# maxwerhahn/Multi-pass-GAN

Measured on AMD Instinct MI355X. Metric: volumes/sec (4x two-pass generator inference, 64^3->256^3 density-only), higher is better.
Workload: dtype f16+2xbf6->f32

## Files before the change

### multi-pass-gan_amd/csrc/mpgan_conv.h

```cpp
#pragma once
#include "mpgan_internal.h"
#include "mpgan_mfma_dev.h"

namespace mpg::conv {

using namespace mpg::dev;

constexpr int TW = 32;
constexpr int TAPOFF_BYTES = 1024;
constexpr int epi_rowf(int nt) { return nt * 32 + 4; }

struct SegArgs {
    const char* x;
    const char* w;
    int cg_seg;
    int cg_total, g_off;
    int kh, kw, up;
    int cgc, nchunks, sc;
    int ih, iw;
    int pt, pl;
    int hs, ws;
    int np;
    int ni_img;
    int direct;
    int tp;
    int pref;
};

struct ConvArgs {
    int n, h, w, cout, nseg;
    SegArgs seg[MPG_MAX_SEG];
    const float* bias;
    int act;
    float leak;
    int pn;
    float pn_eps;
    const float* post_add;
    int pa_stride, pa_coff;
    float* y;
    char* y_g8;
    const float* in_amax;
    const char* zeros;
    int img_bytes;
    int tap_bytes;
    int tiles_x, tiles_y;
    int dbg;
};

typedef const __attribute__((address_space(4))) ConvArgs* KArgs;

struct ConvArgsD2S {
    ConvArgs a;
    int cs;
    int coff;
    int cg;
};
typedef const __attribute__((address_space(4))) ConvArgsD2S* KArgsD2S;

template <bool D2S>
struct KernelArgs { typedef ConvArgs type; };
template <>
struct KernelArgs<true> { typedef ConvArgsD2S type; };

struct D2SPos {
    int cc;
    size_t pix;
};
__device__ __forceinline__ D2SPos d2s_pos(const KArgsD2S dp, int py, int px, int c) {
    const int gc = dp->coff + c;
    const int k = gc / dp->cs;
    D2SPos p;
    p.cc = gc - k * dp->cs;
    p.pix = (size_t)(2 * py + (k >> 1)) * (2 * dp->a.w) + 2 * px + (k & 1);
    return p;
}

template <int NT, int PREC>
struct Pipe {
    static constexpr int WAVES = 4;
    static constexpr int NPL = (PREC == 3) ? 2 : 1;
    static constexpr int PT = (NT >= 3) ? 2 : 4;
    static constexpr int TH = 4 * PT;
    static constexpr int KS = (PREC == 3) ? ((NT == 4 || NT == 2) ? 1 : 2) : ((NT == 4 || NT == 2) ? 2 : 4);
    static constexpr int R = (NT == 3) ? 3 : 4;
    static constexpr int D = R - 1;
    static constexpr int WPLANE = KS * NT * 1024;
    static constexpr int WSTAGE = WPLANE * NPL;
    static constexpr int NI = WSTAGE / 4096;
    static constexpr int ROWF = epi_rowf(NT);
    static_assert(WSTAGE % 4096 == 0, "stage must be a whole number of 256 x 16-byte pieces");
};

template <int NT>
struct Pipe6 {
    static constexpr int WAVES = (NT == 1) ? 4 : 8;
    static constexpr int PT = 16 / WAVES;
    static constexpr int TH = 16;
    static constexpr int KS = 4;
    static constexpr int WF16 = KS * NT * 1024;
    static constexpr int WF6 = NT * 2048;
    static constexpr int WSTAGE = WF16 + 2 * WF6;
    static constexpr int R = 3;
    static constexpr int D = R - 1;
    static constexpr int NI = WSTAGE / (WAVES * 1024);
    static constexpr int ROWF = epi_rowf(NT);
    static_assert(WSTAGE % (WAVES * 1024) == 0, "stage must be a whole number of per-wave pieces");
};

struct EpiPre {
    float bias;
    float amax;
};
__device__ __forceinline__ EpiPre epilogue_prefetch(const KArgs ap, int tid) {
    const auto& a = *ap;
    EpiPre pre;
    pre.bias = (a.bias != nullptr && tid < a.cout) ? a.bias[tid] : 0.f;
    pre.amax = a.in_amax != nullptr ? *a.in_amax : 0.f;
    return pre;
}

template <int ACT, int NT>
__device__ __forceinline__ void epilogue_bias_act(f32x16 (&acc)[NT], const float* bl, float* stg_lane, float unscale, float leak, int cout,
                                                  int hh) {
    if constexpr (ACT == MPG_ACT_TANH) {
#pragma unroll
        for (int nt = 0; nt < NT; ++nt)
#pragma unroll
            for (int q4 = 0; q4 < 4; ++q4) {
                const int co0 = nt * 32 + 8 * q4 + 4 * hh;
                const float4 bq = *reinterpret_cast<const float4*>(bl + co0);
                *reinterpret_cast<float4*>(stg_lane + co0) =
                    make_float4(acc[nt][4 * q4] * unscale + bq.x, acc[nt][4 * q4 + 1] * unscale + bq.y,
                                acc[nt][4 * q4 + 2] * unscale + bq.z, acc[nt][4 * q4 + 3] * unscale + bq.w);
            }
#pragma nounroll
        for (int k = 0; k < NT * 16; ++k) {
            const int c = (k >> 2) * 8 + 4 * hh + (k & 3);
            stg_lane[c] = c < cout ? tanhf(stg_lane[c]) : 0.f;
        }
#pragma unroll
        for (int nt = 0; nt < NT; ++nt)
#pragma unroll
            for (int q4 = 0; q4 < 4; ++q4) {
                const float4 v = *reinterpret_cast<const float4*>(stg_lane + nt * 32 + 8 * q4 + 4 * hh);
                acc[nt][4 * q4] = v.x;
                acc[nt][4 * q4 + 1] = v.y;
                acc[nt][4 * q4 + 2] = v.z;
                acc[nt][4 * q4 + 3] = v.w;
            }
        return;
    }
    float4 bq[2][4];
#pragma unroll
    for (int q4 = 0; q4 < 4; ++q4) bq[0][q4] = *reinterpret_cast<const float4*>(bl + 8 * q4 + 4 * hh);
#pragma unroll
    for (int nt = 0; nt < NT; ++nt) {
        if (nt + 1 < NT) {
#pragma unroll
            for (int q4 = 0; q4 < 4; ++q4) bq[(nt + 1) & 1][q4] = *reinterpret_cast<const float4*>(bl + (nt + 1) * 32 + 8 * q4 + 4 * hh);
        }
        __builtin_amdgcn_sched_barrier(0);
#pragma unroll
        for (int q4 = 0; q4 < 4; ++q4) {
            const int co0 = nt * 32 + 8 * q4 + 4 * hh;
            const float b4[4] = {bq[nt & 1][q4].x, bq[nt & 1][q4].y, bq[nt & 1][q4].z, bq[nt & 1][q4].w};
#pragma unroll
            for (int i = 0; i < 4; ++i) {
                float v = mpg::apply_act(acc[nt][4 * q4 + i] * unscale + b4[i], ACT, leak);
                if (co0 + i >= cout) v = 0.f;
                acc[nt][4 * q4 + i] = v;
            }
        }
        __builtin_amdgcn_sched_barrier(0);
    }
}

template <int NT>
__device__ __forceinline__ void epilogue_row_values(f32x16 (&acc)[NT], const KArgs ap, const float* bl, float* stg_lane, float unscale,
                                                    int hh) {
    const auto& a = *ap;
    switch (a.act) {
        case MPG_ACT_RELU: epilogue_bias_act<MPG_ACT_RELU>(acc, bl, stg_lane, unscale, a.leak, a.cout, hh); break;
        case MPG_ACT_LRELU: epilogue_bias_act<MPG_ACT_LRELU>(acc, bl, stg_lane, unscale, a.leak, a.cout, hh); break;
        case MPG_ACT_TANH: epilogue_bias_act<MPG_ACT_TANH>(acc, bl, stg_lane, unscale, a.leak, a.cout, hh); break;
        default: epilogue_bias_act<MPG_ACT_NONE>(acc, bl, stg_lane, unscale, a.leak, a.cout, hh); break;
    }
    if (a.pn) {
        float ss = 0.f;
#pragma unroll
        for (int nt = 0; nt < NT; ++nt)
#pragma unroll
            for (int i = 0; i < 16; ++i) ss += acc[nt][i] * acc[nt][i];
        ss += __shfl_xor(ss, 32);
        const float sc = rsqrtf(ss / (float)a.cout + a.pn_eps);
#pragma unroll
        for (int nt = 0; nt < NT; ++nt)
#pragma unroll
            for (int i = 0; i < 16; ++i) acc[nt][i] *= sc;
    }
}

template <int NT, int PT, bool D2S = false>
__device__ __forceinline__ void conv_epilogue(f32x16 (&acc)[PT][NT], const KArgs ap, char* smem, int n, int y0, int x0,
                                              int wave, int lane, const EpiPre pre) {
    const auto& a = *ap;
    const KArgsD2S dp = reinterpret_cast<KArgsD2S>(ap);
    const int r = lane & 31;
    const int hh = lane >> 5;
    constexpr int ROWF = epi_rowf(NT);
    static_assert(128 * sizeof(float) <= TAPOFF_BYTES, "the staged bias must fit in front of the staging rows");
    float* bl = reinterpret_cast<float*>(smem);
    float* stg = reinterpret_cast<float*>(smem + TAPOFF_BYTES) + wave * (32 * ROWF);
    const int cg_out = (a.cout + 7) >> 3;
    const float unscale = 1.f / mpg::pow2_scale(pre.amax);
    {
        float bv = pre.bias;
        asm volatile("" : "+v"(bv));
        if (wave < 2) bl[wave * 64 + lane] = bv;
    }
    __syncthreads();
    const int npx = min(32, a.w - x0);
    const size_t plane_px = (size_t)a.h * a.w;
    if (a.y == nullptr && a.post_add == nullptr) {
#pragma unroll
        for (int pt = 0; pt < PT; ++pt) {
            const int py = y0 + PT * wave + pt;
            epilogue_row_values<NT>(acc[pt], ap, bl, stg + r * ROWF, unscale, hh);
            if (py < a.h && r < npx && !(a.dbg & 2)) {
#pragma unroll
                for (int nt = 0; nt < NT; ++nt)
#pragma unroll
                    for (int qp = 0; qp < 2; ++qp) {
                        float v[8];
#pragma unroll
                        for (int i = 0; i < 4; ++i) {
                            typedef unsigned v2u_t __attribute__((ext_vector_type(2)));
                            const v2u_t sw = __builtin_amdgcn_permlane32_swap(__float_as_uint(acc[pt][nt][8 * qp + i]),
                                                                              __float_as_uint(acc[pt][nt][8 * qp + 4 + i]), false, false);
                            v[i] = __uint_as_float(sw[0]);
                            v[4 + i] = __uint_as_float(sw[1]);
                        }
                        const int cg = nt * 4 + 2 * qp + hh;
                        if (cg < cg_out) {
                            char* dst;
                            size_t plane_out = plane_px;
                            if constexpr (D2S) {
                                const D2SPos q = d2s_pos(dp, py, x0 + r, 8 * cg);
                                plane_out = 4 * plane_px;
                                dst = a.y_g8 + ((((size_t)n * dp->cg + (q.cc >> 3)) * 2) * plane_out + q.pix) * 16;
                            } else {
                                dst = a.y_g8 + ((((size_t)n * cg_out + cg) * 2) * plane_px + (size_t)py * a.w + x0 + r) * 16;
                            }
                            half8 hi, lo;
#pragma unroll
                            for (int j = 0; j < 8; ++j) {
                                hi[j] = (_Float16)v[j];
                                lo[j] = (_Float16)(v[j] - (float)hi[j]);
                            }
                            __builtin_nontemporal_store(hi, reinterpret_cast<half8*>(dst));
                            __builtin_nontemporal_store(lo, reinterpret_cast<half8*>(dst + plane_out * 16));
                        }
                    }
            }
        }
        return;
    }
#pragma unroll
    for (int pt = 0; pt < PT; ++pt) {
        const int py = y0 + PT * wave + pt;
        epilogue_row_values<NT>(acc[pt], ap, bl, stg + r * ROWF, unscale, hh);
#pragma unroll
        for (int nt = 0; nt < NT; ++nt)
#pragma unroll
            for (int q4 = 0; q4 < 4; ++q4) {
                const int co0 = nt * 32 + 8 * q4 + 4 * hh;
                *reinterpret_cast<float4*>(stg + r * ROWF + co0) =
                    make_float4(acc[pt][nt][4 * q4], acc[pt][nt][4 * q4 + 1], acc[pt][nt][4 * q4 + 2], acc[pt][nt][4 * q4 + 3]);
            }
        if (py < a.h && !(a.dbg & 2)) {
            const size_t pix0 = ((size_t)n * a.h + py) * a.w + x0;
            if (a.post_add != nullptr) {
                const float* pa = a.post_add + pix0 * a.pa_stride + a.pa_coff;
                const int total = npx * a.cout;
                for (int f0 = lane; f0 < total; f0 += 256) {
                    float pv[4];
                    int so[4];
#pragma unroll
                    for (int j = 0; j < 4; ++j) {
                        const int f = min(f0 + 64 * j, total - 1);
                        const int p = f / a.cout;
                        const int c = f - p * a.cout;
                        so[j] = p * ROWF + c;
                        pv[j] = pa[(size_t)p * a.pa_stride + c];
                    }
#pragma unroll
                    for (int j = 0; j < 4; ++j) {
                        asm volatile("" : "+v"(pv[j]));
                        if (f0 + 64 * j < total) stg[so[j]] += pv[j];
                    }
                }
            }
            if (D2S && a.y != nullptr) {
                float* img = a.y + (size_t)n * 4 * a.h * a.w * dp->cs;
                const int total = npx * a.cout;
                if (((dp->cs | dp->coff | a.cout) & 3) == 0) {
                    for (int f = lane * 4; f < total; f += 256) {
                        const int p = f / a.cout;
                        const int c = f - p * a.cout;
                        const D2SPos q = d2s_pos(dp, py, x0 + p, c);
                        *reinterpret_cast<float4*>(img + q.pix * dp->cs + q.cc) = *reinterpret_cast<const float4*>(stg + p * ROWF + c);
                    }
                } else {
                    for (int f = lane; f < total; f += 64) {
                        const int p = f / a.cout;
                        const int c = f - p * a.cout;
                        const D2SPos q = d2s_pos(dp, py, x0 + p, c);
                        img[q.pix * dp->cs + q.cc] = stg[p * ROWF + c];
                    }
                }
            } else if (a.y != nullptr) {
                float* dst = a.y + pix0 * a.cout;
                const int total = npx * a.cout;
                if ((a.cout & 3) == 0) {
                    for (int f = lane * 4; f < total; f += 256) {
                        const int p = f / a.cout;
                        const int c = f - p * a.cout;
                        *reinterpret_cast<float4*>(dst + f) = *reinterpret_cast<const float4*>(stg + p * ROWF + c);
                    }
                } else {
                    for (int f = lane; f < total; f += 64) {
                        const int p = f / a.cout;
                        dst[f] = stg[p * ROWF + (f - p * a.cout)];
                    }
                }
            }
            if (a.y_g8 != nullptr) {
                if (r < npx) {
                    for (int cg = hh; cg < cg_out; cg += 2) {
                        const float4 v0 = *reinterpret_cast<const float4*>(stg + r * ROWF + cg * 8);
                        const float4 v1 = *reinterpret_cast<const float4*>(stg + r * ROWF + cg * 8 + 4);
                        const float v[8] = {v0.x, v0.y, v0.z, v0.w, v1.x, v1.y, v1.z, v1.w};
                        char* dst;
                        size_t plane_out = plane_px;
                        if constexpr (D2S) {
                            const D2SPos q = d2s_pos(dp, py, x0 + r, 8 * cg);
                            plane_out = 4 * plane_px;
                            dst = a.y_g8 + ((((size_t)n * dp->cg + (q.cc >> 3)) * 2) * plane_out + q.pix) * 16;
                        } else {
                            dst = a.y_g8 + ((((size_t)n * cg_out + cg) * 2) * plane_px + (size_t)py * a.w + x0 + r) * 16;
                        }
                        half8 hi, lo;
#pragma unroll
                        for (int j = 0; j < 8; ++j) {
                            hi[j] = (_Float16)v[j];
                            lo[j] = (_Float16)(v[j] - (float)hi[j]);
                        }
                        __builtin_nontemporal_store(hi, reinterpret_cast<half8*>(dst));
                        __builtin_nontemporal_store(lo, reinterpret_cast<half8*>(dst + plane_out * 16));
                    }
                }
            }
        }
    }
}

struct Shape {
    int th;
    int ks;
    int waves;
    int wstage;
    int ring;
    int rowf;
};
const Shape& pipe_shape(int nt, int prec);

struct SegShape {
    int cgc, nchunks, sc, np, ni_img, img_bytes, direct, tp, pref;
    int slots;
    int stages;
};
SegShape seg_shape(int kh, int kw, int cin, int nt, int prec);

constexpr size_t LDS_MAX = 160 * 1024;

size_t pack_base_bytes(int kh, int kw, int cin, int cout, int prec);
inline bool small_layer(int cin, int cout) { return cin <= 8 && cout <= 8; }
inline int pad_before(int k, int pad_hi) { return pad_hi ? k / 2 : (k - 1) / 2; }
int check_segment(const mpg_conv_desc* d, int s);

hipError_t launch_conv_f16(int prec, int nt, dim3 grid, size_t lds, hipStream_t st, const ConvArgs& a);
hipError_t launch_conv_f16(int prec, int nt, dim3 grid, size_t lds, hipStream_t st, const ConvArgsD2S& a);
hipError_t launch_conv_f6(int nt, dim3 grid, size_t lds, hipStream_t st, const ConvArgs& a);
int launch_small(hipStream_t stream, const mpg_conv_desc* d);

}
```

### multi-pass-gan_amd/csrc/mpgan_conv_f6.hip

```cpp
#include "mpgan_conv.h"

using namespace mpg::conv;

namespace {

#ifndef MPG_AH
#define MPG_AH 2
#endif
#ifndef MPG_WD
#define MPG_WD 1
#endif
#ifndef MPG_DIAG6
#define MPG_DIAG6 0
#endif
#ifndef MPG_W0
#define MPG_W0 1
#endif
#ifndef MPG_IMG_LATE
#define MPG_IMG_LATE 0
#endif
#ifndef MPG_PIECES_AFTER
#define MPG_PIECES_AFTER 1
#endif
#ifndef MPG_ALT
#define MPG_ALT 0
#endif
#ifndef MPG_STAMPS
#define MPG_STAMPS 0
#endif
#if MPG_STAMPS
#define MPG_STAMP(v) asm volatile("s_memtime %0" : "=s"(v))
#else
#define MPG_STAMP(v)
#endif
constexpr int lo_step(int pt, int nt, int ptn) {
    const int s = nt - ptn + pt - 1;
    return s < 0 ? 0 : (s > nt - 1 ? nt - 1 : s);
}

typedef int v16i __attribute__((ext_vector_type(16)));
typedef int v8i __attribute__((ext_vector_type(8)));
typedef int v6i __attribute__((ext_vector_type(6)));
typedef _Float16 half32 __attribute__((ext_vector_type(32)));
typedef _Float16 half16 __attribute__((ext_vector_type(16)));

__device__ __forceinline__ v8i lds_read32(const char* p) {
    const v4i lo = *reinterpret_cast<const v4i*>(p);
    const v4i hi = *reinterpret_cast<const v4i*>(p + 1024);
    return __builtin_shufflevector(lo, hi, 0, 1, 2, 3, 4, 5, 6, 7);
}

template <int OFF, class T>
__device__ __forceinline__ void ds_read16(T& dst, unsigned addr) {
    static_assert(sizeof(T) == 16 && OFF >= 0 && OFF < 65536, "one ds_read_b128");
    asm volatile("ds_read_b128 %0, %1 offset:%2" : "=v"(dst) : "v"(addr), "n"(OFF));
}

constexpr int kx_cum(int h, int NT, int PT) { return h + PT * ((h + NT - 1) / NT); }
constexpr int kx_allowed(int g, int NT, int PT, int AH) {
    const int G16 = 4 * NT;
    const int hi = g + AH + 1 < G16 ? g + AH + 1 : G16;
    return kx_cum(hi, NT, PT) - kx_cum(g + 1, NT, PT);
}

__device__ __forceinline__ half32 cat32(const half8& a, const half8& b, const half8& c, const half8& d) {
    const half16 lo = __builtin_shufflevector(a, b, 0, 1, 2, 3, 4, 5, 6, 7, 8, 9, 10, 11, 12, 13, 14, 15);
    const half16 hi = __builtin_shufflevector(c, d, 0, 1, 2, 3, 4, 5, 6, 7, 8, 9, 10, 11, 12, 13, 14, 15);
    return __builtin_shufflevector(lo, hi, 0, 1, 2, 3, 4, 5, 6, 7, 8, 9, 10, 11, 12, 13, 14, 15, 16, 17, 18, 19, 20, 21, 22, 23,
                                   24, 25, 26, 27, 28, 29, 30, 31);
}

__device__ __forceinline__ int block_exp16(const half32& v) {
    const v16i r = __builtin_bit_cast(v16i, v);
    int a0, a1, a2, a3, a4, a5, a6, a7, b0, b1, b2, b3, b4, b5, b6, b7, m2, m1;
#define MPG_MAX3(d, x, y, z) asm("v_pk_maximum3_f16 %0, %1, %2, %3" : "=v"(d) : "v"(x), "v"(y), "v"(z))
#define MPG_MIN3(d, x, y, z) asm("v_pk_minimum3_f16 %0, %1, %2, %3" : "=v"(d) : "v"(x), "v"(y), "v"(z))
    MPG_MAX3(a0, r[0], r[1], r[2]); MPG_MAX3(a1, r[3], r[4], r[5]); MPG_MAX3(a2, r[6], r[7], r[8]); MPG_MAX3(a3, r[9], r[10], r[11]);
    MPG_MAX3(a4, r[12], r[13], r[14]); MPG_MAX3(a5, a0, a1, r[15]); MPG_MAX3(a6, a2, a3, a4); MPG_MAX3(a7, a5, a6, a6);
    MPG_MIN3(b0, r[0], r[1], r[2]); MPG_MIN3(b1, r[3], r[4], r[5]); MPG_MIN3(b2, r[6], r[7], r[8]); MPG_MIN3(b3, r[9], r[10], r[11]);
    MPG_MIN3(b4, r[12], r[13], r[14]); MPG_MIN3(b5, b0, b1, r[15]); MPG_MIN3(b6, b2, b3, b4); MPG_MIN3(b7, b5, b6, b6);
#undef MPG_MAX3
#undef MPG_MIN3
    asm("v_pk_max_f16 %0, %1, %2 neg_lo:[0,1] neg_hi:[0,1]" : "=v"(m2) : "v"(a7), "v"(b7));
    asm("v_pk_max_f16 %0, %1, %1 op_sel:[0,1] op_sel_hi:[1,0]" : "=v"(m1) : "v"(m2));
    return (m1 >> 10) & 31;
}

#ifndef MPG_CVT_DIVIDES
#define MPG_CVT_DIVIDES 1
#endif
__device__ __forceinline__ float pow2_from_byte(int e8m0) {
#if MPG_CVT_DIVIDES
    return __builtin_bit_cast(float, e8m0 << 23);
#else
    return __builtin_bit_cast(float, (254 - e8m0) << 23);
#endif
}
__device__ __forceinline__ v8i widen6(const v6i& v) {
    return __builtin_shufflevector(v, v, 0, 1, 2, 3, 4, 5, -1, -1);
}
__device__ __forceinline__ v8i bf6_of(const half32& v, int e8m0) {
    return widen6(__builtin_amdgcn_cvt_scalef32_pk32_bf6_f16(v, pow2_from_byte(e8m0)));
}
constexpr int BF6 = 3;

template <int NT>
__global__ __launch_bounds__(Pipe6<NT>::WAVES * 64, 2) void conv_mfma_f6_kernel(const ConvArgs a_unused) {
    extern __shared__ __attribute__((aligned(16))) char smem[];
    const KArgs ap = (KArgs)__builtin_amdgcn_kernarg_segment_ptr();
    const auto& a = *ap;
    using P = Pipe6<NT>;
    constexpr int WAVES = P::WAVES, PT = P::PT, TH = P::TH, WF16 = P::WF16, WF6 = P::WF6, WSTAGE = P::WSTAGE;
    constexpr int NI = P::NI, R = P::R, D = P::D, THREADS = WAVES * 64;

    int* tap16 = reinterpret_cast<int*>(smem);
    char* img_lds = smem + a.tap_bytes;
    char* w_lds = img_lds + 2 * a.img_bytes;

    const int tid = threadIdx.x;
    const int lane = tid & 63;
    const int wave = tid >> 6;
    const int wave_u = __builtin_amdgcn_readfirstlane(wave);
    const int r = lane & 31;
    const int hh = lane >> 5;

    int bid = blockIdx.x;
    const int nblk = gridDim.x;
    if ((nblk & 7) == 0) bid = (bid & 7) * (nblk >> 3) + (bid >> 3);
    const int tx = bid % a.tiles_x;
    const int t2 = bid / a.tiles_x;
    const int ty = t2 % a.tiles_y;
    const int n = t2 / a.tiles_y;
    const int y0 = ty * TH, x0 = tx * TW;

    f32x16 acc[PT][NT];
#pragma unroll
    for (int pt = 0; pt < PT; ++pt)
#pragma unroll
        for (int nt = 0; nt < NT; ++nt)
#pragma unroll
            for (int i = 0; i < 16; ++i) acc[pt][nt][i] = 0.f;

    const EpiPre pre = epilogue_prefetch(ap, tid);
    const int seg_flip = (NT == 1 && a.nseg > 1) ? ((int)(blockIdx.x >> 8) & 1) : 0;
    for (int s0 = 0; s0 < ((a.dbg & 1) ? 0 : a.nseg); ++s0) {
        const int s = seg_flip ? a.nseg - 1 - s0 : s0;
        const auto& sg = ap->seg[s];
        if (NT <= 2 && sg.direct) {
            const unsigned plane_bytes = (unsigned)(sg.hs * sg.ws) * 16u;
            const unsigned gstride = 2u * plane_bytes;
            const char* xb = sg.x + ((size_t)n * sg.cg_total + sg.g_off) * gstride;
            unsigned pixo[PT];
#pragma unroll
            for (int pt = 0; pt < PT; ++pt) {
                int yy = y0 + PT * wave + pt, xx = x0 + r;
                yy = (yy < a.h ? yy : a.h - 1) >> sg.up;
                xx = (xx < a.w ? xx : a.w - 1) >> sg.up;
                pixo[pt] = (unsigned)(yy * sg.ws + xx) * 16u;
            }
            const int glast = sg.cg_seg - 1;
            auto dma_stage_d = [&](int stage) {
                const int sidx = stage < sg.sc ? stage : sg.sc - 1;
                const char* src = sg.w + (size_t)sidx * WSTAGE + tid * 16;
                char* dst = w_lds + (stage % R) * WSTAGE + wave_u * 1024;
#pragma unroll
                for (int i = 0; i < NI; ++i) dma16(src + i * (THREADS * 16), dst + i * (THREADS * 16));
            };
#pragma unroll
            for (int d = 0; d < D; ++d) dma_stage_d(d);
            for (int st = 0; st < sg.sc; ++st) {
                wait_dma_and_barrier<(D - 1) * NI>();
                dma_stage_d(st + D);
                const char* wb = w_lds + (st % R) * WSTAGE;
                const char* xs = xb + (size_t)st * 8 * gstride;
                const int grem = glast - st * 8;
                constexpr int PH = PT == 4 ? 1 : 2;
                static_for<0, PT / PH>([&](auto hc) {
                    constexpr int p0 = decltype(hc)::value * PH;
                    half8 b_hi[4][PH], b_lo[4][PH];
#pragma unroll
                    for (int j = 0; j < 4; ++j) {
                        int g = 2 * j + hh;
                        g = g < grem ? g : grem;
#pragma unroll
                        for (int q = 0; q < PH; ++q) {
                            b_hi[j][q] = __builtin_nontemporal_load(reinterpret_cast<const half8*>(xs + (pixo[p0 + q] + g * gstride)));
                            b_lo[j][q] = __builtin_nontemporal_load(reinterpret_cast<const half8*>(xs + (pixo[p0 + q] + g * gstride + plane_bytes)));
                        }
                    }
#pragma unroll
                    for (int j = 0; j < 4; ++j) {
#pragma unroll
                        for (int nt = 0; nt < NT; ++nt) {
                            const half8 a_hi = *reinterpret_cast<const half8*>(wb + ((j * NT + nt) * 64 + lane) * 16);
#pragma unroll
                            for (int q = 0; q < PH; ++q)
                                acc[p0 + q][nt] = __builtin_amdgcn_mfma_f32_32x32x16_f16(a_hi, b_hi[j][q], acc[p0 + q][nt], 0, 0, 0);
                        }
                    }
                    v8i hi6[PH], lo6[PH];
                    int sb[PH];
#pragma unroll
                    for (int q = 0; q < PH; ++q) {
                        const half32 bh = cat32(b_hi[0][q], b_hi[1][q], b_hi[2][q], b_hi[3][q]);
                        const half32 bl = cat32(b_lo[0][q], b_lo[1][q], b_lo[2][q], b_lo[3][q]);
                        const int e = block_exp16(bh);
                        hi6[q] = bf6_of(bh, e + 109);
                        lo6[q] = bf6_of(bl, e + 97);
                        sb[q] = (e + 109) | (e + 97) << 8;
                    }
#pragma unroll
                    for (int nt = 0; nt < NT; ++nt) {
                        const v8i w_hi = lds_read32(wb + WF16 + nt * 2048 + lane * 16);
                        const v8i w_lo = lds_read32(wb + WF16 + WF6 + nt * 2048 + lane * 16);
#pragma unroll
                        for (int q = 0; q < PH; ++q) {
                            acc[p0 + q][nt] = __builtin_amdgcn_mfma_scale_f32_32x32x64_f8f6f4(w_lo, hi6[q], acc[p0 + q][nt], BF6, BF6, 1, w_lo[6], 0, sb[q]);
                            acc[p0 + q][nt] = __builtin_amdgcn_mfma_scale_f32_32x32x64_f8f6f4(w_hi, lo6[q], acc[p0 + q][nt], BF6, BF6, 0, w_hi[6], 1, sb[q]);
                        }
                    }
                });
            }
            asm volatile("s_waitcnt vmcnt(0)" ::: "memory");
            __syncthreads();
            continue;
        }
        const int T = sg.kh * sg.kw;
        const int G = sg.nchunks;
        const int NS = sg.sc;
        const int plane_b = sg.np * 16;
        const int ppg = sg.np >> 6;

        for (int q = tid; q < NS * 8; q += THREADS) {
            const int g = q / sg.tp;
            const int t = q - g * sg.tp;
            int off = ((g < G ? g : G - 1) & 1) * a.img_bytes;
            if (g < G && t < T) {
                const int dy = t / sg.kw;
                const int dx = t - dy * sg.kw;
                off += (dy * sg.iw + dx) * 16;
            }
            tap16[(q >> 3) * 8 + (q & 1) * 4 + ((q & 7) >> 1)] = off;
        }
        int pixb[PT];
#pragma unroll
        for (int pt = 0; pt < PT; ++pt) pixb[pt] = ((PT * wave + pt) * sg.iw + r) * 16;

        const size_t plane_px = (size_t)sg.hs * sg.ws;
        constexpr int MAXI = (WAVES == 8) ? 4 : 7;
        int img_src[MAXI];
#pragma unroll
        for (int i = 0; i < MAXI; ++i) {
            const int pc = WAVES * i + wave_u;
            const int pl = pc / ppg;
            const int p = (pc - pl * ppg) * 64 + lane;
            const int hy = p / sg.iw;
            const int hx = p - hy * sg.iw;
            const int yy = y0 - sg.pt + hy;
            const int xx = x0 - sg.pl + hx;
            const bool ok = pl < 2 && hy < sg.ih && yy >= 0 && yy < a.h && xx >= 0 && xx < a.w;
            img_src[i] = ok ? (int)(((size_t)pl * plane_px + (size_t)(yy >> sg.up) * sg.ws + (xx >> sg.up)) * 16) : -1;
        }
        const size_t group_bytes = 2 * plane_px * 16;
        const char* const x_first = sg.x + ((size_t)n * sg.cg_total + sg.g_off) * group_bytes;
        auto img_piece = [&](int chunk, auto ic) {
            constexpr int i = decltype(ic)::value;
            if ((MPG_DIAG6 & 4) && chunk > 0) return;
            if (i < sg.ni_img) {
                const int off = img_src[i];
                const char* src = (off >= 0 && chunk < sg.cg_seg) ? x_first + (size_t)chunk * group_bytes + off : a.zeros;
                dma16_stream(src, img_lds + (chunk & 1) * a.img_bytes + (WAVES * i + wave_u) * 1024);
            }
        };
        auto w_piece = [&](int stage, auto ic) {
            constexpr int i = decltype(ic)::value;
            const int sidx = stage < NS ? stage : NS - 1;
            if ((MPG_DIAG6 & 8) && stage >= D) return;
            dma16(sg.w + (size_t)sidx * WSTAGE + tid * 16 + i * (THREADS * 16),
                  w_lds + (stage % R) * WSTAGE + wave_u * 1024 + i * (THREADS * 16));
        };
        static_for<0, MAXI>([&](auto ic) { img_piece(0, ic); });
#pragma unroll
        for (int d = 0; d < D; ++d) static_for<0, NI>([&](auto ic) { w_piece(d, ic); });
        int g_next = 1;

        half8 bh[PT][4];
        v4i o16n = {0, 0, 0, 0};
        const unsigned i_base = lds_off(img_lds);
#if MPG_STAMPS
        unsigned long long ts0 = 0, ts1 = 0, ts2 = 0, ts3 = 0, ts3_prev = 0;
        unsigned sum_head = 0, sum_f16 = 0, sum_f6 = 0, sum_bar = 0;
#endif

        auto run_stages = [&](auto oc) {
        constexpr bool CORR_FIRST = decltype(oc)::value != 0;
        int img_in_flight = 0;
        for (int st = 0; st < NS; ++st) {
            if constexpr (MPG_IMG_LATE) wait_dma_rt((D - 1) * NI, img_in_flight);
            else wait_dma_and_barrier<(D - 1) * NI>();
#if MPG_STAMPS
            if (st > 0) {
                sum_head += (unsigned)(ts1 - ts0);
                sum_f16 += (unsigned)(ts2 - ts1);
                sum_f6 += (unsigned)(ts3 - ts2);
                if (st > 1) sum_bar += (unsigned)(ts0 - ts3_prev);
                ts3_prev = ts3;
            }
            MPG_STAMP(ts0);
#endif
            if (st == 0) {
                ds_read16<0>(o16n, lds_off(tap16 + hh * 4));
                lgkm_wait<0>();
            }
            tie(o16n);
            const v4i o16 = o16n;
            const int to16[4] = {o16.x, o16.y, o16.z, o16.w};
            {
                const int sn = st + 1 < NS ? st + 1 : st;
                ds_read16<0>(o16n, lds_off(tap16 + (sn * 2 + hh) * 4));
            }
            const bool do_img = g_next < G && st * 8 >= (g_next - 1) * sg.tp;
            const int img_chunk = g_next;
            img_in_flight = (MPG_IMG_LATE && do_img && (g_next * sg.tp) / 8 >= st + 2) ? sg.ni_img : 0;
            if (do_img) ++g_next;
            const char* wb = w_lds + (st % R) * WSTAGE;
            const unsigned a_base = lds_off(wb) + (unsigned)lane * 16u;
            constexpr int AH = MPG_AH, G16 = 4 * NT;
            half8 aq[AH + 1];
            v8i hi6[PT], lo6[PT];
            int sb[PT], e16[PT];
            auto read_group = [&](auto gc) {
                constexpr int g = decltype(gc)::value, j = g / NT;
                if constexpr (g % NT == 0)
                    static_for<0, PT>([&](auto pc) {
                        constexpr int pt = decltype(pc)::value;
                        ds_read16<0>(bh[pt][j], i_base + (unsigned)(pixb[pt] + to16[j]));
                    });
                ds_read16<g * 1024>(aq[g % (AH + 1)], a_base);
            };
            auto make_hi6 = [&](auto pc) {
                constexpr int pt = decltype(pc)::value;
#if MPG_DIAG6 & 2
                const v4i q0 = __builtin_bit_cast(v4i, bh[pt][0]), q1 = __builtin_bit_cast(v4i, bh[pt][1]);
                hi6[pt] = __builtin_shufflevector(q0, q1, 0, 1, 2, 3, 4, 5, 6, 7);
                e16[pt] = 15;
                sb[pt] = 0x7f7f7f7f;
#else
                const half32 b32 = cat32(bh[pt][0], bh[pt][1], bh[pt][2], bh[pt][3]);
                e16[pt] = block_exp16(b32);
                hi6[pt] = bf6_of(b32, e16[pt] + 109);
                sb[pt] = (e16[pt] + 109) | (e16[pt] + 97) << 8;
#endif
            };
            constexpr int HALF = G16 / 2;
            constexpr int IPG = (MAXI + HALF - 1) / HALF;
            constexpr int WPG = (NI + HALF - 1) / HALF;
            constexpr int KS6 = 2 * NT;
            constexpr int WD = MPG_WD < KS6 - 1 ? MPG_WD : KS6 - 1;
            v4i wq[WD + 1][2];
            auto read_w6 = [&](auto kc) {
                constexpr int k = decltype(kc)::value;
                constexpr int off = WF16 + (k < NT ? WF6 + k * 2048 : (k - NT) * 2048);
                ds_read16<off>(wq[k % (WD + 1)][0], a_base);
                ds_read16<off + 1024>(wq[k % (WD + 1)][1], a_base);
            };
            auto fp16_phase = [&](auto mk) {
                constexpr bool MAKE_HI6 = decltype(mk)::value != 0;
                constexpr bool W0_AHEAD = MAKE_HI6 && MPG_W0;
                static_for<0, (AH < G16 ? AH : G16)>([&](auto gc) { read_group(gc); });
                static_for<0, G16>([&](auto gc) {
                    constexpr int g = decltype(gc)::value, j = g / NT, nt = g % NT;
                    auto pieces = [&]() {
                        if constexpr (g < HALF) {
                            if (do_img)
                                static_for<0, IPG>([&](auto kc) {
                                    constexpr int i = g * IPG + decltype(kc)::value;
                                    if constexpr (i < MAXI) img_piece(img_chunk, std::integral_constant<int, i>{});
                                });
                        } else {
                            static_for<0, WPG>([&](auto kc) {
                                constexpr int i = (g - HALF) * WPG + decltype(kc)::value;
                                if constexpr (i < NI) w_piece(st + D, std::integral_constant<int, i>{});
                            });
                        }
                    };
                    if constexpr (!MPG_PIECES_AFTER) pieces();
                    if constexpr (g + AH < G16) read_group(std::integral_constant<int, g + AH>{});
                    if constexpr (W0_AHEAD && g == G16 - 1) read_w6(std::integral_constant<int, 0>{});
                    lgkm_wait<kx_allowed(g, NT, PT, AH) + (W0_AHEAD && g == G16 - 1 ? 2 : 0)>();
                    if constexpr (g == 0 && MAKE_HI6) { MPG_STAMP(ts1); }
                    tie(aq[g % (AH + 1)]);
                    if constexpr (nt == 0)
                        static_for<0, PT>([&](auto pc) { tie(bh[decltype(pc)::value][j]); });
                    static_for<0, PT>([&](auto pc) {
                        constexpr int pt = decltype(pc)::value;
                        acc[pt][nt] = __builtin_amdgcn_mfma_f32_32x32x16_f16(aq[g % (AH + 1)], bh[pt][j], acc[pt][nt], 0, 0, 0);
                    });
                    if constexpr (MPG_PIECES_AFTER) pieces();
                    if constexpr (MAKE_HI6) {
                        if constexpr (g >= 3 * NT && g - 3 * NT < PT) make_hi6(std::integral_constant<int, g - 3 * NT>{});
                        if constexpr (g == G16 - 1 && NT < PT) static_for<NT, PT>([&](auto pc) { make_hi6(pc); });
                    }
                });
            };
            auto bf6_phase = [&](auto w0c) {
            constexpr bool W0_DONE = decltype(w0c)::value != 0;
#if !(MPG_DIAG6 & 1)
            constexpr int PB = PT;
            auto read_bl = [&](auto pc) {
                constexpr int pt = decltype(pc)::value;
                static_for<0, 4>([&](auto jc) {
                    constexpr int j = decltype(jc)::value;
                    ds_read16<0>(bh[pt][j], i_base + (unsigned)(plane_b + pixb[pt] + to16[j]));
                });
            };
            auto make_lo6 = [&](auto pc) {
                constexpr int pt = decltype(pc)::value;
                static_for<0, 4>([&](auto jc) { tie(bh[pt][decltype(jc)::value]); });
#if MPG_DIAG6 & 2
                const v4i q0 = __builtin_bit_cast(v4i, bh[pt][0]), q1 = __builtin_bit_cast(v4i, bh[pt][1]);
                lo6[pt] = __builtin_shufflevector(q0, q1, 0, 1, 2, 3, 4, 5, 6, 7);
#else
                lo6[pt] = bf6_of(cat32(bh[pt][0], bh[pt][1], bh[pt][2], bh[pt][3]), e16[pt] + 97);
#endif
            };
            if constexpr (!W0_DONE) read_w6(std::integral_constant<int, 0>{});
            static_for<0, PB>([&](auto pc) { read_bl(pc); });
            static_for<1, WD + 1>([&](auto kc) { read_w6(kc); });
            static_for<0, KS6>([&](auto kc) {
                constexpr int k = decltype(kc)::value;
                if constexpr (k >= 1 && k + WD < KS6) read_w6(std::integral_constant<int, k + WD>{});
                constexpr int ahead = (k + WD < KS6 ? k + WD : KS6 - 1) - k;
                lgkm_wait<(k == 0 ? 4 * PB : 0) + 2 * ahead>();
                tie(wq[k % (WD + 1)][0]);
                tie(wq[k % (WD + 1)][1]);
                const v8i w6 = __builtin_shufflevector(wq[k % (WD + 1)][0], wq[k % (WD + 1)][1], 0, 1, 2, 3, 4, 5, 6, 7);
                static_for<0, PT>([&](auto pc) {
                    constexpr int pt = decltype(pc)::value;
                    if constexpr (k < NT)
                        acc[pt][k] = __builtin_amdgcn_mfma_scale_f32_32x32x64_f8f6f4(w6, hi6[pt], acc[pt][k], BF6, BF6, 1, w6[6], 0, sb[pt]);
                    else
                        acc[pt][k - NT] = __builtin_amdgcn_mfma_scale_f32_32x32x64_f8f6f4(w6, lo6[pt], acc[pt][k - NT], BF6, BF6, 0, w6[6], 1, sb[pt]);
                });
                if constexpr (k < NT) {
                    if constexpr (k == 0 && lo_step(0, NT, PT) == 0) lgkm_wait<2 * ahead>();
                    static_for<0, PT>([&](auto pc) {
                        if constexpr (lo_step(decltype(pc)::value, NT, PT) == k) make_lo6(pc);
                    });
                }
            });
#else
            const v8i& h0 = hi6[0];
            const int &s0 = sb[0], &e0 = e16[0];
            asm volatile("" ::"v"(h0), "v"(s0), "v"(e0));
#endif
            };
            if constexpr (CORR_FIRST) {
                static_for<0, PT>([&](auto pc) {
                    constexpr int pt = decltype(pc)::value;
                    static_for<0, 4>([&](auto jc) {
                        constexpr int j = decltype(jc)::value;
                        ds_read16<0>(bh[pt][j], i_base + (unsigned)(pixb[pt] + to16[j]));
                    });
                });
                lgkm_wait<0>();
                static_for<0, PT>([&](auto pc) {
                    static_for<0, 4>([&](auto jc) { tie(bh[decltype(pc)::value][decltype(jc)::value]); });
                    make_hi6(pc);
                });
                MPG_STAMP(ts1);
                bf6_phase(std::integral_constant<int, 0>{});
                MPG_STAMP(ts2);
                fp16_phase(std::integral_constant<int, 0>{});
            } else {
                fp16_phase(std::integral_constant<int, 1>{});
                MPG_STAMP(ts2);
                bf6_phase(std::integral_constant<int, MPG_W0>{});
            }
            MPG_STAMP(ts3);
        }
        };
#if MPG_ALT
        if (WAVES == 8 && wave_u >= WAVES / 2) run_stages(std::integral_constant<int, 1>{});
        else
#endif
            run_stages(std::integral_constant<int, 0>{});
        asm volatile("s_waitcnt vmcnt(0) lgkmcnt(0)" ::: "memory");
        __syncthreads();
#if MPG_STAMPS
        if ((a.dbg & 8) && a.y != nullptr && s == 0 && lane == 0) {
            unsigned* o = reinterpret_cast<unsigned*>(a.y) + ((size_t)blockIdx.x * WAVES + wave) * 4;
            o[0] = sum_head; o[1] = sum_f16; o[2] = sum_f6; o[3] = sum_bar;
        }
#endif
    }
    conv_epilogue<NT, PT>(acc, ap, smem, n, y0, x0, wave, lane, pre);
}

}

hipError_t mpg::conv::launch_conv_f6(int nt, dim3 grid, size_t lds, hipStream_t st, const ConvArgs& a) {
    switch (nt) {
        case 1: return mpg::launch_dyn_lds<conv_mfma_f6_kernel<1>>(grid, dim3(Pipe6<1>::WAVES * 64), lds, st, a);
        case 2: return mpg::launch_dyn_lds<conv_mfma_f6_kernel<2>>(grid, dim3(Pipe6<2>::WAVES * 64), lds, st, a);
        case 3: return mpg::launch_dyn_lds<conv_mfma_f6_kernel<3>>(grid, dim3(Pipe6<3>::WAVES * 64), lds, st, a);
        default: return mpg::launch_dyn_lds<conv_mfma_f6_kernel<4>>(grid, dim3(Pipe6<4>::WAVES * 64), lds, st, a);
    }
}
```

Baseline: 15.26.

## Run NT=1 bf6 conv kernel with 8 waves, occupancy 4, and a flat pipelined inner loop

For NT=1, the f6 conv kernel now uses 8 waves per block instead of 4 (PT drops from 4 to 2) and requests 4 blocks per CU through a new OCC constant. The direct path gets a hand-scheduled inner loop that interleaves explicit LDS reads with f16 and scaled bf6 MFMAs under fine-grained lgkm waits, so weight-fragment loads overlap compute. The goal is more latency hiding and less register pressure per wave. Tighter launch bounds risk register spills, and the new control-flow around the direct segment (continue placement under FLAT) adds complexity.

```diff
diff --git a/multi-pass-gan_amd/csrc/mpgan_conv.h b/multi-pass-gan_amd/csrc/mpgan_conv.h
--- a/multi-pass-gan_amd/csrc/mpgan_conv.h
+++ b/multi-pass-gan_amd/csrc/mpgan_conv.h
@@ -93,7 +93,8 @@
 
 template <int NT>
 struct Pipe6 {
-    static constexpr int WAVES = (NT == 1) ? 4 : 8;
+    static constexpr int WAVES = 8;
+    static constexpr int OCC = (NT == 1) ? 4 : 2;
     static constexpr int PT = 16 / WAVES;
     static constexpr int TH = 16;
     static constexpr int KS = 4;
diff --git a/multi-pass-gan_amd/csrc/mpgan_conv_f6.hip b/multi-pass-gan_amd/csrc/mpgan_conv_f6.hip
--- a/multi-pass-gan_amd/csrc/mpgan_conv_f6.hip
+++ b/multi-pass-gan_amd/csrc/mpgan_conv_f6.hip
@@ -105,13 +105,14 @@
 constexpr int BF6 = 3;
 
 template <int NT>
-__global__ __launch_bounds__(Pipe6<NT>::WAVES * 64, 2) void conv_mfma_f6_kernel(const ConvArgs a_unused) {
+__global__ __launch_bounds__(Pipe6<NT>::WAVES * 64, Pipe6<NT>::OCC) void conv_mfma_f6_kernel(const ConvArgs a_unused) {
     extern __shared__ __attribute__((aligned(16))) char smem[];
     const KArgs ap = (KArgs)__builtin_amdgcn_kernarg_segment_ptr();
     const auto& a = *ap;
     using P = Pipe6<NT>;
     constexpr int WAVES = P::WAVES, PT = P::PT, TH = P::TH, WF16 = P::WF16, WF6 = P::WF6, WSTAGE = P::WSTAGE;
     constexpr int NI = P::NI, R = P::R, D = P::D, THREADS = WAVES * 64;
+    constexpr bool FLAT = NT == 1;
 
     int* tap16 = reinterpret_cast<int*>(smem);
     char* img_lds = smem + a.tap_bytes;
@@ -174,7 +175,60 @@
                 const char* wb = w_lds + (st % R) * WSTAGE;
                 const char* xs = xb + (size_t)st * 8 * gstride;
                 const int grem = glast - st * 8;
-                constexpr int PH = PT == 4 ? 1 : 2;
+                if constexpr (FLAT) {
+                    const unsigned a_base = lds_off(wb) + (unsigned)lane * 16u;
+                    const char* xs_hi = xs;
+                    const char* xs_lo = xs + plane_bytes;
+                    asm volatile("" : "+s"(xs_hi), "+s"(xs_lo));
+                    static_for<0, PT>([&](auto qc) {
+                        constexpr int q = decltype(qc)::value;
+                        half8 b_hi[4], b_lo[4], aq[2];
+                        v4i wl[2], wh[2];
+#pragma unroll
+                        for (int j = 0; j < 4; ++j) {
+                            int g = 2 * j + hh;
+                            g = g < grem ? g : grem;
+                            const unsigned vo = pixo[q] + g * gstride;
+                            typedef const __attribute__((address_space(1))) half8* gmem;
+                            b_hi[j] = __builtin_nontemporal_load((gmem)(xs_hi + vo));
+                            b_lo[j] = __builtin_nontemporal_load((gmem)(xs_lo + vo));
+                        }
+                        ds_read16<0>(aq[0], a_base);
+                        ds_read16<1024>(aq[1], a_base);
+                        static_for<0, 4>([&](auto jc) {
+                            constexpr int j = decltype(jc)::value;
+                            lgkm_wait<(j < 3 ? 1 : 2)>();
+                            tie(aq[j & 1]);
+                            acc[q][0] = __builtin_amdgcn_mfma_f32_32x32x16_f16(aq[j & 1], b_hi[j], acc[q][0], 0, 0, 0);
+                            if constexpr (j < 2) {
+                                ds_read16<(j + 2) * 1024>(aq[j & 1], a_base);
+                            } else if constexpr (j == 2) {
+                                ds_read16<WF16 + WF6>(wl[0], a_base);
+                                ds_read16<WF16 + WF6 + 1024>(wl[1], a_base);
+                            } else {
+                                ds_read16<WF16>(wh[0], a_base);
+                                ds_read16<WF16 + 1024>(wh[1], a_base);
+                            }
+                        });
+                        const half32 bh = cat32(b_hi[0], b_hi[1], b_hi[2], b_hi[3]);
+                        const int e = block_exp16(bh);
+                        const v8i hi6 = bf6_of(bh, e + 109);
+                        const v8i lo6 = bf6_of(cat32(b_lo[0], b_lo[1], b_lo[2], b_lo[3]), e + 97);
+                        const int sb = (e + 109) | (e + 97) << 8;
+                        lgkm_wait<2>();
+                        tie(wl[0]);
+                        tie(wl[1]);
+                        const v8i w_lo = __builtin_shufflevector(wl[0], wl[1], 0, 1, 2, 3, 4, 5, 6, 7);
+                        acc[q][0] = __builtin_amdgcn_mfma_scale_f32_32x32x64_f8f6f4(w_lo, hi6, acc[q][0], BF6, BF6, 1, w_lo[6], 0, sb);
+                        lgkm_wait<0>();
+                        tie(wh[0]);
+                        tie(wh[1]);
+                        const v8i w_hi = __builtin_shufflevector(wh[0], wh[1], 0, 1, 2, 3, 4, 5, 6, 7);
+                        acc[q][0] = __builtin_amdgcn_mfma_scale_f32_32x32x64_f8f6f4(w_hi, lo6, acc[q][0], BF6, BF6, 0, w_hi[6], 1, sb);
+                    });
+                    continue;
+                }
+                constexpr int PH = 2;
                 static_for<0, PT / PH>([&](auto hc) {
                     constexpr int p0 = decltype(hc)::value * PH;
                     half8 b_hi[4][PH], b_lo[4][PH];
@@ -223,7 +277,10 @@
             }
             asm volatile("s_waitcnt vmcnt(0)" ::: "memory");
             __syncthreads();
-            continue;
+            if constexpr (!FLAT) continue;
+        }
+        if constexpr (FLAT) {
+            if (__builtin_amdgcn_readfirstlane(sg.direct)) continue;
         }
         const int T = sg.kh * sg.kw;
         const int G = sg.nchunks;
@@ -247,7 +304,8 @@
         for (int pt = 0; pt < PT; ++pt) pixb[pt] = ((PT * wave + pt) * sg.iw + r) * 16;
 
         const size_t plane_px = (size_t)sg.hs * sg.ws;
-        constexpr int MAXI = (WAVES == 8) ? 4 : 7;
+        constexpr int MAXI = 4;
+        static_assert(WAVES == 8, "MAXI");
         int img_src[MAXI];
 #pragma unroll
         for (int i = 0; i < MAXI; ++i) {
```

New measurement: 15.49, median of 6. 1.5% higher.
